# sailist/emotion-recognition-in-conversation

Measured on AMD Instinct MI355X. Metric: utterances/sec training step, COGMEN IEMOCAP-6 atv, higher is better.
Workload: dtype bf16

## Files before the change

emotion-recognition-in-conversation_amd/capi.py:

```python
import ctypes as C
import os
import re
import subprocess

import torch

_HERE = os.path.dirname(os.path.abspath(__file__))
LIB_PATH = os.environ.get("ERC_LIB_PATH") or os.path.join(_HERE, "lib", "libercgraft.so")
CSRC = os.path.join(_HERE, "csrc")
HEADER = os.path.join(os.path.dirname(_HERE), "include", "ercgraft.h")


class ErcGraftError(RuntimeError):
    pass


_CTYPES = {"int": C.c_int, "int32_t": C.c_int, "int64_t": C.c_int64, "uint64_t": C.c_uint64, "float": C.c_float}


def _ctype(decl, proto, ret=False):
    t = " ".join(decl.replace("*", " * ").split())
    if ret and t == "const char *":
        return C.c_char_p
    if "*" in t:
# ... 1100 lines not shown
    return list(order)[:n_nodes]


def chain_build(raw_graph):
    handle = int(lib().erc_chain_build(raw_graph))
    return (handle, None) if handle else (0, lib().erc_last_error().decode())


def chain_len(chain):
    n = int(lib().erc_chain_len(chain))
    if n < 0:
        _check(n, "erc_chain_len")
    return n


def chain_run(chain):
    _check(lib().erc_chain_run(chain, stream()), "erc_chain_run")


def chain_free(chain):
    _check(lib().erc_chain_free(chain), "erc_chain_free")
```

emotion-recognition-in-conversation_amd/csrc/cogmen_fused.hip:

```cpp
#include "erc_common.h"
#include "split_dev.h"

namespace {

typedef float f32x4 __attribute__((ext_vector_type(4)));
typedef short bf16x8 __attribute__((ext_vector_type(8)));

constexpr int CG_F = 100;
constexpr int CG_R = 8;
constexpr int CG_HL = 5;
constexpr int CG_TR = 16;
constexpr int CG_MID = CG_TR + 2 * CG_HL;
constexpr int CG_OUT = CG_TR + 4 * CG_HL;
constexpr int CG_FAR = CG_TR + 6 * CG_HL;
constexpr int CG_KM = (CG_R + 1) * CG_F;
constexpr int CG_KMP = 928;
constexpr int CG_SM = 936;
constexpr int CG_SH1 = 136;
constexpr int CG_SQ = 404;
constexpr int CG_CH = 12;
constexpr int CG_NT = 7;

constexpr int CG_NW = 16;
constexpr int CG_NTH = 64 * CG_NW;
// ... 103 lines not shown
    int* bn_counter;
    float* running_mean;
    float* running_var;
    float* saved;
    float momentum, eps, scale;
    int N, ldh0, ldmb, ldh1b, ldh2, bn_fused, two_spk;
    const int32_t* n_dev;
    int32_t* health;
    int32_t* events;
    uint64_t* stamps;
    int stamp_block;
    int64_t catT_plane, q_plane;
    float* Mf;
    float* H1f;
    int ldmf, ldh1f;
};

template <int NT>
__global__ __launch_bounds__(CG_NTH) void cogmen_fwd_tile_kernel(const CgFwdP p) {
    constexpr bool X = NT > 1;
    using XM = FxMap<X ? NT : 2>;
    if (p.health && blockIdx.x == 0 && threadIdx.x == 0 && *p.health != 0) {
        p.events[0] += 1;
        *p.health = 0;
    }
    extern __shared__ __attribute__((aligned(16))) unsigned char lds[];
    unsigned short* const sM = reinterpret_cast<unsigned short*>(lds + (X ? XM::SM_OFF : FW_SM_OFF));
    float* const sQ = reinterpret_cast<float*>(lds + (X ? XM::SM_OFF : FW_SM_OFF));
    unsigned short* const sH1 = reinterpret_cast<unsigned short*>(lds + (X ? XM::SH1_OFF : FW_SH1_OFF));
    float* const sH0 = reinterpret_cast<float*>(lds + (X ? XM::SH0_OFF : FW_SH0_OFF));
// ... 159 lines not shown
                            const int grp = (q >> 2) * 2 + (q & 1);
                            *reinterpret_cast<float2*>(grow + q * CG_F) = ((q >> 1) & 1) == a ? mq[grp] : make_float2(0.f, 0.f);
                        }
                        *reinterpret_cast<float2*>(grow + CG_R * CG_F) = self;
                    }
                }
            }
            uint32_t* const mrow = reinterpret_cast<uint32_t*>(sM + e * CG_SM);
            uint32_t* const grow = reinterpret_cast<uint32_t*>(p.Mb + (int64_t)(own ? node : 0) * p.ldmb);
            if (!X && act) {
#pragma unroll
                for (int q = 0; q < CG_R; ++q) {
                    const int grp = (q >> 2) * 2 + (q & 1);
                    const uint32_t v = ((q >> 1) & 1) == a ? pk4[grp] : 0u;
                    mrow[q * (CG_F / 2) + lane] = v;
                    if (own) grow[q * (CG_F / 2) + lane] = v;
                }
                mrow[CG_R * (CG_F / 2) + lane] = pks;
                if (own) grow[CG_R * (CG_F / 2) + lane] = pks;
            }
            if (own && lane < CG_R) {
                const int grp = (lane >> 2) * 2 + (lane & 1);
                int c = 0;
#pragma unroll
                for (int q = 0; q < 4; ++q) c = grp == q ? cnt[q] : c;
                c = ((lane >> 1) & 1) == a ? c : 0;
                p.inv_cnt[(int64_t)node * CG_R + lane] = c > 0 ? 1.0f / (float)c : 0.f;
            }
        }
    } else
    {
        const bool act = lane < CG_F / 2;
        const int c2 = 2 * min(lane, CG_F / 2 - 1);
#pragma unroll 1
// ... 24 lines not shown
            float2 self = *reinterpret_cast<const float2*>(sH0 + le * CG_F + c2);
            if (!valid) self = make_float2(0.f, 0.f);
            const bool own = valid && e >= CG_HL && e < CG_HL + CG_TR;
            uint32_t* const mrow = reinterpret_cast<uint32_t*>(sM + e * CG_SM);
            uint32_t* const grow = reinterpret_cast<uint32_t*>(p.Mb + (int64_t)(own ? node : 0) * p.ldmb);
            const float fc_l = (float)max(cnt_l, 1), rc_l = __builtin_amdgcn_rcpf(fc_l);
#pragma unroll
            for (int q = 0; q < CG_R; ++q) {
                const float fc = __builtin_bit_cast(float, __builtin_amdgcn_readlane(__builtin_bit_cast(int, fc_l), q));
                const float rc = __builtin_bit_cast(float, __builtin_amdgcn_readlane(__builtin_bit_cast(int, rc_l), q));
                float m0 = s0[q] * rc, m1 = s1[q] * rc;
                m0 = fmaf(fmaf(-m0, fc, s0[q]), rc, m0), m1 = fmaf(fmaf(-m1, fc, s1[q]), rc, m1);
                const uint32_t pk = (uint32_t)f2bf(m0) | ((uint32_t)f2bf(m1) << 16);
                if (act) {
                    mrow[q * (CG_F / 2) + lane] = pk;
                    if (own) grow[q * (CG_F / 2) + lane] = pk;
                }
            }
            const uint32_t pks = (uint32_t)f2bf(self.x) | ((uint32_t)f2bf(self.y) << 16);
            if (act) {
                mrow[CG_R * (CG_F / 2) + lane] = pks;
                if (own) grow[CG_R * (CG_F / 2) + lane] = pks;
            }
            if (own && lane < CG_R) p.inv_cnt[(int64_t)node * CG_R + lane] = cnt_l > 0 ? 1.0f / (float)cnt_l : 0.f;
        }
    }
    __syncthreads();
    CG_STAMP(2);

    f32x4 acc0 = {0.f, 0.f, 0.f, 0.f}, acc1 = {0.f, 0.f, 0.f, 0.f};
    if (mma_wave) {
        if constexpr (!X) {
            const unsigned short* const a0 = sM + r * CG_SM + 8 * g + 32 * KH0 * kh;
            const unsigned short* const a1 = sM + min(16 + r, 26) * CG_SM + 8 * g + 32 * KH0 * kh;
#pragma unroll
            for (int u = 0; u < KH0; ++u) {
                if (u < nkb) {
// ... 63 lines not shown
    if (mma_wave && !kh) {
        const float* src = sPart + (ct * 64 + lane) * 8;
        const f32x4 p0 = *reinterpret_cast<const f32x4*>(src), p1 = *reinterpret_cast<const f32x4*>(src + 4);
        const int col = 16 * ct + r;
        const float bias = p.b1[min(col, CG_F - 1)];
#pragma unroll
        for (int h = 0; h < 2; ++h)
#pragma unroll
            for (int i = 0; i < 4; ++i) {
                const int e = 16 * h + 4 * g + i;
                const float v = (h ? acc1[i] + p1[i] : acc0[i] + p0[i]) + bias;
                const int node = mb + e;
                if constexpr (!X) {
                    const unsigned short hb = col < CG_F ? f2bf(v) : (unsigned short)0;
                    sH1[e * CG_SH1 + col] = hb;
                    if (col < CG_F && e >= CG_HL && e < CG_HL + CG_TR && node < N) p.H1b[(int64_t)node * p.ldh1b + col] = hb;
                } else {
                    float rem = col < CG_F ? v : 0.f;
#pragma unroll
                    for (int t = 0; t < NT; ++t) {
                        const __bf16 hb = (__bf16)rem;
                        rem -= (float)hb;
                        sH1[t * (FW_SH1_BYTES / 2) + e * CG_SH1 + col] = __builtin_bit_cast(unsigned short, hb);
                    }
                    if (col < CG_F && e >= CG_HL && e < CG_HL + CG_TR && node < N) p.H1f[(int64_t)node * p.ldh1f + col] = v;
                }
            }
    } else if (w == 7) {
        for (int i = lane; i < 32 * 16 * NT; i += 64) sH1[(i >> 9) * (FW_SH1_BYTES / 2) + ((i >> 4) & 31) * CG_SH1 + 112 + (i & 15)] = 0;
    }
    __syncthreads();
    CG_STAMP(3);

    {
        bf16x8 fa[X ? 1 : 2][4];
        if constexpr (!X) {
#pragma unroll
            for (int h = 0; h < 2; ++h)
#pragma unroll
                for (int kb = 0; kb < 4; ++kb) fa[h][kb] = *reinterpret_cast<const bf16x8*>(sH1 + (16 * h + r) * CG_SH1 + 32 * kb + 8 * g);
        }
#pragma unroll
        for (int j = 0; j < 2; ++j) {
            const int qt = w + 16 * j;
            f32x4 acc[2] = {{0.f, 0.f, 0.f, 0.f}, {0.f, 0.f, 0.f, 0.f}};
            if constexpr (X) {
                const unsigned short* const bq1 = p.Wq + ((int64_t)min(w + 16, 24) * 4 * 64 + lane) * 8;
// ... 31 lines not shown
                        const int e = 16 * h + 4 * g + i;
                        if (e < CG_MID) sQ[e * CG_SQ + 16 * qt + r] = acc[h][i] + qbias[j];
                    }
            }
        }
    }
    __syncthreads();
    CG_STAMP(4);

#pragma unroll
    for (int j = 0; j < 2; ++j) {
        const int i = tid + CG_NTH * j;
        const int li = i / 100, q = i % 100;
        const int node = r0 + li;
        if (i < CG_TR * 100 && node < N)
            *reinterpret_cast<f32x4*>(p.QKVS + (int64_t)node * 400 + 4 * q) = *reinterpret_cast<const f32x4*>(sQ + (CG_HL + li) * CG_SQ + 4 * q);
    }

    {
        const bool act = lane < CG_F / 2;
        const int c2 = 2 * min(lane, CG_F / 2 - 1);
        const float am = act ? 1.f : 0.f;
        const int li = w, node = r0 + li, e = CG_HL + li;
        const bool valid = node < N;
        const int e0 = __builtin_amdgcn_readfirstlane(max(sIp[e] - E_lo, 0));
        const int nwin = __builtin_amdgcn_readfirstlane(valid ? min(max(sIp[e + 1] - sIp[e], 0), CG_CH) : 0);
        float2 qv = *reinterpret_cast<const float2*>(sQ + e * CG_SQ + c2);
        qv.x *= am, qv.y *= am;
        const float2 sk = *reinterpret_cast<const float2*>(sQ + e * CG_SQ + 3 * CG_F + c2);
        int ljs[CG_CH];
#pragma unroll
// ... 13 lines not shown
        for (int u = 0; u < CG_CH; ++u) {
            sc[u] *= p.scale;
            if (u < nwin) mx = fmaxf(mx, sc[u]);
        }
#pragma unroll
        for (int u = 0; u < CG_CH; ++u) {
            const float pw = u < nwin ? expf(sc[u] - mx) : 0.f;
            sc[u] = pw;
            den += pw;
            o0 += pw * vv[u].x, o1 += pw * vv[u].y;
        }
        const float inv = 1.0f / (den + 1e-16f);
        const float2 y = make_float2(valid ? o0 * inv + sk.x : 0.f, valid ? o1 * inv + sk.y : 0.f);
        if (act) *reinterpret_cast<float2*>(sH2 + li * CG_F + c2) = y;
        if (valid) {
            if (act) *reinterpret_cast<float2*>(p.H2 + (int64_t)node * p.ldh2 + c2) = y;
            float mine = 0.f;
#pragma unroll
            for (int u = 0; u < CG_CH; ++u)
                if (lane == u) mine = sc[u];
            if (lane < nwin) p.alpha[sIp[e] + lane] = mine * inv;
        }
    }
    CG_STAMP(5);
    if (!p.bn_fused) return;

    __syncthreads();
    if (tid < 2 * CG_F) {
        const int c = tid % CG_F, sq = tid / CG_F;
        double s = 0.0;
#pragma unroll
        for (int li = 0; li < CG_TR; ++li) {
            const double x = (double)sH2[li * CG_F + c];
            s += sq ? x * x : x;
        }
        if (p.bn_fused == 2) {
            reinterpret_cast<float*>(p.bn_part)[(int64_t)blockIdx.x * 2 * CG_F + tid] = (float)s;
        } else {
            st_sc1d(p.bn_part + (int64_t)blockIdx.x * 2 * CG_F + tid, s);
        }
    }
    if (p.bn_fused == 2) {
// ... 123 lines not shown
    float* dgamma;
    float* dbeta;
    float* stats;
    int head_parts, hp_floats;
    const unsigned short* WqT;
    const unsigned short* Wb;
    float* dQKVS;
    float* dH1;
    float* dH0;
    float scale;
    int N, ldh2, lddh0, lddh1, grads_bf16, two_spk;
    const int32_t* n_dev;
    uint64_t* stamps;
    int stamp_block;
    int64_t qT_plane, wb_plane;
};

template <int NT>
__global__ __launch_bounds__(CG_NTH) void cogmen_bwd_tile_kernel(const CgBwdP p) {
    constexpr bool X = NT > 1;
    using XM = BxMap<X ? NT : 2>;
    extern __shared__ __attribute__((aligned(16))) unsigned char lds[];
    float* const sK = reinterpret_cast<float*>(lds + (X ? XM::SK_OFF : BW_SK_OFF));
    float* const sV = reinterpret_cast<float*>(lds + (X ? XM::SV_OFF : BW_SV_OFF));
    float* const sQq = reinterpret_cast<float*>(lds + (X ? XM::SQ_OFF : BW_SQ_OFF));
    float* const sG = reinterpret_cast<float*>(lds + (X ? XM::SG_OFF : BW_SG_OFF));
    float* const sAl = reinterpret_cast<float*>(lds + (X ? XM::SE_OFF : BW_SE_OFF));
    int* const sSrc = reinterpret_cast<int*>(sAl + 2 * BW_ECAP);
    int* const sOd = sSrc + BW_ECAP;
    int* const sOt = sOd + 2 * BW_OCAP;
// ... 222 lines not shown
#pragma unroll
        for (int j = 0; j < 2; ++j) {
            const int i = tid + CG_NTH * j;
            const int em = i / 50, cp = i % 50;
            if (i < CG_MID * 50) {
                const float2 gv = *reinterpret_cast<const float2*>(sG + (em + CG_HL) * CG_F + 2 * cp);
                if constexpr (!X) {
                    sDQw[em * (CG_SDQ / 2) + 150 + cp] = (uint32_t)f2bf(gv.x) | ((uint32_t)f2bf(gv.y) << 16);
                } else {
                    unsigned tt[NT];
                    sp_split2<NT>(gv.x, gv.y, tt);
#pragma unroll
                    for (int t = 0; t < NT; ++t) sDQw[t * DQPW + em * (CG_SDQ / 2) + 150 + cp] = tt[t];
                }
                const int node = mb + em;
                if (em >= CG_HL && em < CG_HL + CG_TR && node < N) {
                    if (p.grads_bf16) *reinterpret_cast<uint32_t*>(reinterpret_cast<unsigned short*>(p.dQKVS) + (int64_t)node * 400 + 3 * CG_F + 2 * cp) = (uint32_t)f2bf(gv.x) | ((uint32_t)f2bf(gv.y) << 16);
                    else *reinterpret_cast<float2*>(p.dQKVS + (int64_t)node * 400 + 3 * CG_F + 2 * cp) = gv;
                }
            }
        }
#pragma unroll
        for (int ui = 0; ui < 3; ++ui) {
            if constexpr (!X) {
#pragma unroll
                for (int t5 = 0; t5 < 5; ++t5) bx[5 * ui + t5] = *reinterpret_cast<const bf16x8*>(brow5 + 512 * (5 * ui + t5));
            }
            const int u = w + CG_NW * ui;
            if (u >= 42) continue;
            const int kind = u < 14 ? 0 : 1 + (u - 14) / 14, uu = u < 14 ? u : (u - 14) % 14;
            const int rt = uu / 7, cti = uu % 7;
// ... 18 lines not shown
                const int node = mb + em;
                const bool rowv = em >= 0 && em < CG_MID;
                if (rowv && 16 * cti + r < CG_F) {
                    const bool nv = node >= 0 && node < N;
                    if constexpr (!X) {
                        sDQ[em * CG_SDQ + coff + 16 * cti + r] = f2bf(nv ? acc[q] : 0.f);
                    } else {
                        float rem = nv ? acc[q] : 0.f;
#pragma unroll
                        for (int t = 0; t < NT; ++t) {
                            const __bf16 hb = (__bf16)rem;
                            rem -= (float)hb;
                            sDQ[t * (BX_DQPLANE / 2) + em * CG_SDQ + coff + 16 * cti + r] = __builtin_bit_cast(unsigned short, hb);
                        }
                    }
                    if (nv && em >= CG_HL && em < CG_HL + CG_TR) {
                        if (p.grads_bf16) reinterpret_cast<unsigned short*>(p.dQKVS)[(int64_t)node * 400 + coff + 16 * cti + r] = f2bf(acc[q]);
                        else p.dQKVS[(int64_t)node * 400 + coff + 16 * cti + r] = acc[q];
                    }
                }
            }
        }
    }
    __syncthreads();
    CG_STAMP(3);

    {
        f32x4 acc0 = {0.f, 0.f, 0.f, 0.f}, acc1 = {0.f, 0.f, 0.f, 0.f};
        if (mma_wave) {
            const unsigned short* const a0 = sDQ + r * CG_SDQ + 8 * g + 32 * 7 * kh;
            if constexpr (!X) {
#pragma unroll
            for (int u = 0; u < 7; ++u) {
                if (u < (kh ? 6 : 7)) {
                    const bf16x8 fa0 = *reinterpret_cast<const bf16x8*>(a0 + 32 * u);
                    const bf16x8 fa1 = *reinterpret_cast<const bf16x8*>(a0 + 16 * CG_SDQ + 32 * u);
                    acc0 = __builtin_amdgcn_mfma_f32_16x16x32_bf16(fa0, fb3[u], acc0, 0, 0, 0);
                    acc1 = __builtin_amdgcn_mfma_f32_16x16x32_bf16(fa1, fb3[u], acc1, 0, 0, 0);
                }
            }
// ... 28 lines not shown
        }
        __syncthreads();
        if (mma_wave && !kh) {
            const float* src = sPart3 + (ct * 64 + lane) * 8;
            const f32x4 p0 = *reinterpret_cast<const f32x4*>(src), p1 = *reinterpret_cast<const f32x4*>(src + 4);
            const int col = 16 * ct + r;
            if (col < CG_F) {
#pragma unroll
                for (int h = 0; h < 2; ++h)
#pragma unroll
                    for (int i = 0; i < 4; ++i) {
                        const int e = 16 * h + 4 * g + i;
                        const float v = h ? acc1[i] + p1[i] : acc0[i] + p0[i];
                        sDH1[e * CG_F + col] = v;
                        const int node = mb + e;
                        if (e >= CG_HL && e < CG_HL + CG_TR && node < N) {
                            if (p.grads_bf16) reinterpret_cast<unsigned short*>(p.dH1)[(int64_t)node * p.lddh1 + col] = f2bf(v);
                            else p.dH1[(int64_t)node * p.lddh1 + col] = v;
                        }
                    }
            }
        }
    }
    __syncthreads();
    CG_STAMP(4);

    {
        const bool act = lane < CG_F / 2;
        const int c2 = 2 * min(lane, CG_F / 2 - 1);
        uint32_t* const sDPw = reinterpret_cast<uint32_t*>(sDP);
        const int li = w, em = CG_HL + li, node = r0 + li;
        const bool valid = node < N;
        const int o0 = __builtin_amdgcn_readfirstlane(sOp[em] - O_lo), o1 = __builtin_amdgcn_readfirstlane(sOp[em + 1] - O_lo);
        const int nwin = valid ? min(max(o1 - o0, 0), CG_CH) : 0;
        const int xb = max(o0, 0);
        const int xm = min(xb + min(lane, max(nwin - 1, 0)), BW_OCAP - 1);
        const int my_off = min(max(sOd[xm] - mb, 0), CG_MID - 1) * CG_F, my_typ = lane < nwin ? sOt[xm] : CG_R;
        const float my_w = sOw[xm];
        float s0[CG_R], s1[CG_R];
#pragma unroll
// ... 183 lines not shown
    p.Wq = (const unsigned short*)Wq; p.bq = bq; p.inv_cnt = inv_cnt;
    if (terms == 1) {
        p.Mb = (unsigned short*)Mb; p.H1b = (unsigned short*)H1b; p.ldmb = ldmb; p.ldh1b = ldh1b;
    } else {
        p.Mf = (float*)Mb; p.H1f = (float*)H1b; p.ldmf = ldmb; p.ldh1f = ldh1b; p.catT_plane = catT_plane; p.q_plane = q_plane;
    }
    p.QKVS = QKVS; p.H2 = H2; p.alpha = alpha;
    const int tiles = erc_cdiv(n_nodes, CG_TR);
    p.bn_part = bn_ws ? bn_ws + 2 : nullptr;
    p.bn_counter = reinterpret_cast<int*>(bn_ws);
    p.running_mean = running_mean; p.running_var = running_var; p.saved = saved;
    p.momentum = momentum; p.eps = eps; p.scale = scale;
    p.N = n_nodes; p.ldh0 = ldh0; p.ldh2 = ldh2; p.bn_fused = bn_fused;
    p.node_spk = node_spk; p.two_spk = n_speakers == 2 ? 1 : 0; p.n_dev = n_dev;
    p.health = health, p.events = events;
    p.stamps = g_cg_stamps; p.stamp_block = tiles / 2;
    if (terms == 1) hipLaunchKernelGGL(cogmen_fwd_tile_kernel<1>, dim3(tiles), dim3(CG_NTH), lds_bytes, (hipStream_t)stream, p);
    else if (terms == 2) hipLaunchKernelGGL(cogmen_fwd_tile_kernel<2>, dim3(tiles), dim3(CG_NTH), lds_bytes, (hipStream_t)stream, p);
    else hipLaunchKernelGGL(cogmen_fwd_tile_kernel<3>, dim3(tiles), dim3(CG_NTH), lds_bytes, (hipStream_t)stream, p);
    ERC_LAUNCH_CHECK("cogmen_fwd_tile");
    return ERC_OK;
}

extern "C" int erc_cogmen_fwd_tile(const float* H0, int ldh0, int n_nodes, int wp, int wf, const int32_t* in_ptr,
                                   const int32_t* in_src, const int32_t* in_typ, const void* WcatT, const float* b1,
                                   const void* Wq, const float* bq, float scale, void* Mb, int ldmb, float* inv_cnt, void* H1b,
                                   int ldh1b, float* QKVS, float* H2, int ldh2, float* alpha, int bn_fused,
                                   float* running_mean, float* running_var, float momentum, float eps, float* saved,
                                   double* bn_ws, const int32_t* node_spk, int n_speakers, const int32_t* n_dev, int32_t* health,
                                   int32_t* events, void* stream) {
// ... 41 lines not shown
    const void* kern = terms == 1 ? reinterpret_cast<const void*>(cogmen_bwd_tile_kernel<1>)
                     : terms == 2 ? reinterpret_cast<const void*>(cogmen_bwd_tile_kernel<2>)
                                  : reinterpret_cast<const void*>(cogmen_bwd_tile_kernel<3>);
    const int lds_bytes = terms == 1 ? BW_LDS : terms == 2 ? BxMap<2>::LDS : BxMap<3>::LDS;
    ERC_REQUIRE(ensure_lds(kern, lds_bytes), "cogmen_bwd_tile: %d bytes of LDS refused", lds_bytes);
    CgBwdP p{};
    p.dY = dY; p.H2 = H2; p.gamma = gamma; p.saved = saved; p.bn_bwd = bn_bwd; p.QKVS = QKVS; p.alpha = alpha;
    p.in_ptr = in_ptr; p.in_src = in_src; p.out_ptr = out_ptr; p.out_dst = out_dst; p.out_typ = out_typ; p.out_eid = out_eid;
    p.inv_cnt = inv_cnt; p.WqT = (const unsigned short*)WqT; p.Wb = (const unsigned short*)Wb;
    p.qT_plane = qT_plane; p.wb_plane = wb_plane;
    p.dQKVS = (float*)dQKVS; p.dH1 = (float*)dH1; p.dH0 = (float*)dH0; p.scale = scale; p.N = n_nodes; p.ldh2 = ldh2; p.lddh0 = lddh0;
    p.lddh1 = lddh1; p.grads_bf16 = grads_bf16;
    p.node_spk = node_spk; p.two_spk = n_speakers == 2 ? 1 : 0; p.n_dev = n_dev;
    p.head_part = head_part; p.head_parts = head_parts; p.hp_floats = head_part_floats; p.bn_bwd_out = const_cast<float*>(bn_bwd);
    p.dgamma = dgamma; p.dbeta = dbeta; p.stats = stats;
    p.stamps = g_cg_stamps; p.stamp_block = erc_cdiv(n_nodes, CG_TR) / 2;
    const dim3 grid(erc_cdiv(n_nodes, CG_TR));
    if (terms == 1) hipLaunchKernelGGL(cogmen_bwd_tile_kernel<1>, grid, dim3(CG_NTH), lds_bytes, (hipStream_t)stream, p);
    else if (terms == 2) hipLaunchKernelGGL(cogmen_bwd_tile_kernel<2>, grid, dim3(CG_NTH), lds_bytes, (hipStream_t)stream, p);
    else hipLaunchKernelGGL(cogmen_bwd_tile_kernel<3>, grid, dim3(CG_NTH), lds_bytes, (hipStream_t)stream, p);
    ERC_LAUNCH_CHECK("cogmen_bwd_tile");
    return ERC_OK;
}

extern "C" int erc_cogmen_bwd_tile(const float* dY, const float* H2, int ldh2, int n_nodes, int wp, int wf, const float* gamma,
                                   const float* saved, const float* bn_bwd, const float* QKVS, const float* alpha,
                                   const int32_t* in_ptr, const int32_t* in_src, const int32_t* out_ptr, const int32_t* out_dst,
                                   const int32_t* out_typ, const int32_t* out_eid, const float* inv_cnt, const void* WqT,
                                   const void* Wb, float scale, void* dQKVS, void* dH1, void* dH0, int lddh0,
                                   const int32_t* node_spk, int n_speakers, const float* head_part, int head_parts,
// ... 21 lines not shown
```

emotion-recognition-in-conversation_amd/csrc/launch_chain.hip:

```cpp
#include <dlfcn.h>

#include <vector>

#include "erc_common.h"

extern "C" int erc_chain_order(int n_nodes, int n_edges, const int32_t* from_host, const int32_t* to_host, int32_t* order_host) {
    ERC_REQUIRE(n_nodes > 0 && order_host != nullptr, "chain_order: n_nodes=%d (need >= 1 and an output array)", n_nodes);
    ERC_REQUIRE(n_edges == n_nodes - 1, "chain_order: %d nodes with %d edges are not one path", n_nodes, n_edges);
    ERC_REQUIRE(n_edges == 0 || (from_host != nullptr && to_host != nullptr), "chain_order: null edge list");
    std::vector<int32_t> next(n_nodes, -1), pred(n_nodes, -1);
    for (int e = 0; e < n_edges; ++e) {
        const int32_t a = from_host[e], b = to_host[e];
        ERC_REQUIRE(a >= 0 && a < n_nodes && b >= 0 && b < n_nodes && a != b, "chain_order: edge %d (%d -> %d) out of range", e, a, b);
        ERC_REQUIRE(next[a] < 0, "chain_order: node %d has two successors (a fork)", a);
        ERC_REQUIRE(pred[b] < 0, "chain_order: node %d has two predecessors (a join)", b);
        next[a] = b;
        pred[b] = a;
    }
    int root = -1, roots = 0;
    for (int i = 0; i < n_nodes; ++i)
        if (pred[i] < 0) {
            root = i;
            ++roots;
        }
// ... 104 lines not shown
            (void)hipGetLastError();
            return ERC_E_LAUNCH;
        }
    }
    return ERC_OK;
}

extern "C" int erc_chain_free(int64_t chain) {
    if (chain == 0) return ERC_OK;
    Chain* c = chain_of(chain);
    ERC_REQUIRE(c != nullptr, "chain_free: not a chain handle");
    c->magic = 0;
    delete c;
    return ERC_OK;
}
```

emotion-recognition-in-conversation_amd/csrc/wgrad_bf16.hip:

```cpp
#include "erc_common.h"
#include "optim_dev.h"
#include "split_dev.h"
#include <string.h>

namespace {

typedef float f32x4 __attribute__((ext_vector_type(4)));
typedef short bf16x8 __attribute__((ext_vector_type(8)));
typedef unsigned int u32x4 __attribute__((ext_vector_type(4)));
typedef unsigned int u32x2 __attribute__((ext_vector_type(2)));
#define ERC_GLOBAL __attribute__((address_space(1)))

constexpr int W2_IDX_CAP = 4096;
constexpr int W2_SLAB = 128 * 64 + 192;
constexpr int W2_MAX_DESC = 16;

struct W2Desc {
    const unsigned short* A;
    const unsigned short* B;
    float* C;
    float* bias_a;
    float* bias_b;
    const int32_t* b_gather;
    const int32_t* k_dev;
    int lda, ldb, ldc, M, N, K;
    int ct, cvec, splits, tiles_n, item_base, n_items, tile_base;
    int kind;
};

struct W2Adam {
    int decoupled, spin_limit;
    float lr, b1, b2, eps, wd, grad_scale;
    float *data, *grad, *m, *v;
    int64_t* state;
    unsigned short* shadow;
    const int32_t* skip;
    int32_t* seq;
    int32_t* health;
    ShadowTab tab;
    int x_world, x_rank, x_spin, x_pad;
    float* x_pub[8];
    int32_t* x_flags[8];
    int64_t* x_epoch;
    int64_t x_npad;
};
static_assert(sizeof(W2Desc) == 112, "W2Desc layout");

__device__ __forceinline__ float ld_sc1(const float* p) { return __hip_atomic_load(p, __ATOMIC_RELAXED, __HIP_MEMORY_SCOPE_AGENT); }
__device__ __forceinline__ void st_sc1(float* p, float v) { __hip_atomic_store(p, v, __ATOMIC_RELAXED, __HIP_MEMORY_SCOPE_AGENT); }
__device__ __forceinline__ void st_sc1_x4(float* p, f32x4 v) {
    asm volatile("global_store_dwordx4 %0, %1, off sc0 sc1\n\ts_nop 1" ::"v"(p), "v"(v) : "memory");
}
__device__ __forceinline__ f32x4 ld_sc1_x4(const float* p) {
    f32x4 v;
    asm volatile("global_load_dwordx4 %0, %1, off sc0 sc1" : "=v"(v) : "v"(p) : "memory");
    return v;
}
__device__ __forceinline__ float bf_lo(unsigned d) { return __builtin_bit_cast(float, d << 16); }
__device__ __forceinline__ float bf_hi(unsigned d) { return __builtin_bit_cast(float, d & 0xffff0000u); }
__device__ __forceinline__ unsigned perm_lo(unsigned x, unsigned y) { return __builtin_amdgcn_perm(y, x, 0x05040100u); }
__device__ __forceinline__ unsigned perm_hi(unsigned x, unsigned y) { return __builtin_amdgcn_perm(y, x, 0x07060302u); }

#define W2_STAMP(slot)                                                                          \
    do {                                                                                        \
        if (stamps && threadIdx.x == 0) stamps[slot] = __builtin_amdgcn_s_memrealtime();        \
    } while (0)

// ... 24 lines not shown
    auto copy_tab = [&]() __attribute__((always_inline)) {
        ShadowTab* const wt = reinterpret_cast<ShadowTab*>(red);
        wt->n = ad.tab.n, wt->flags = ad.tab.flags;
#pragma unroll
        for (int t = 0; t < SHADOW_MAX; ++t) {
            const ShadowDesc& a = ad.tab.d[t];
            ShadowDesc& b = wt->d[t];
            b.src_off = a.src_off, b.n_el = a.n_el, b.dst_off = a.dst_off, b.n0 = a.n0, b.n1 = a.n1, b.sn0 = a.sn0, b.sn1 = a.sn1;
            b.sn2 = a.sn2, b.sk0 = a.sk0, b.sk1 = a.sk1, b.sk2 = a.sk2, b.ld = a.ld, b.mode = a.mode;
            b.plane_stride = a.plane_stride, b.terms = a.terms;
        }
    };
    auto adam_quad = [&](const int64_t off, const f32x4 gq, const f32x4 pq, const f32x4 mq, const f32x4 vq) __attribute__((always_inline)) -> float4 {
        float4 pv = make_float4(pq.x, pq.y, pq.z, pq.w), mv = make_float4(mq.x, mq.y, mq.z, mq.w), vv = make_float4(vq.x, vq.y, vq.z, vq.w);
        ac.upd(pv.x, gq.x, mv.x, vv.x), ac.upd(pv.y, gq.y, mv.y, vv.y), ac.upd(pv.z, gq.z, mv.z, vv.z), ac.upd(pv.w, gq.w, mv.w, vv.w);
        *(ERC_GLOBAL f32x4*)(ad.data + off) = (f32x4){pv.x, pv.y, pv.z, pv.w};
        *(ERC_GLOBAL f32x4*)(ad.m + off) = (f32x4){mv.x, mv.y, mv.z, mv.w}, *(ERC_GLOBAL f32x4*)(ad.v + off) = (f32x4){vv.x, vv.y, vv.z, vv.w};
        return pv;
    };
    auto shadow_quads = [&](const int64_t (&offs)[8], const float4 (&pn)[8], const int count, const bool (&isq)[8], const unsigned tmask) __attribute__((always_inline)) {
        if (!ad.shadow) return;
        const bool quads = (stab.flags & 1) != 0;
        const int nt = stab.n;
#pragma unroll
        for (int o = 0; o < 8; ++o) {
            if (o >= count || !isq[o]) continue;
            const int64_t i0 = offs[o];
            const float4 pv = pn[o];
#pragma unroll 1
            for (int t = 0; t < nt; ++t) {
                if (!((tmask >> t) & 1)) continue;
                const ShadowDesc& sd = stab.d[t];
// ... 410 lines not shown
                        *reinterpret_cast<f32x4*>(red + w * 4096 + (((hh * 2 + il) * 4 + q) * 64 + lane) * 4) = v * wsel;
                    }
            __syncthreads();
    #pragma unroll
            for (int u = 0; u < 4; ++u) {
                const int f4 = tid + 256 * u;
                f32x4 s = *reinterpret_cast<const f32x4*>(red + f4 * 4);
    #pragma unroll
                for (int ww = 1; ww < 4; ++ww) {
                    const f32x4 t = *reinterpret_cast<const f32x4*>(red + ww * 4096 + f4 * 4);
                    s += t;
                }
                if (direct) {
                    store_c(tid + 256 * (u & 1), 2 * P + (u >> 1), s);
                } else {
                    st_sc1_x4(slab + ((4 * P + u) * 256 + tid) * 4, s);
                }
            }
        }
        if (tid < 192) {
            const float v = ((bred[tid] + bred[192 + tid]) + bred[384 + tid]) + bred[576 + tid];
            if (direct) {
                if (tid < 128) {
                    if (want_a && tid < d.M) ((ERC_GLOBAL float*)d.bias_a)[tid] = v;
                } else if (want_b && n0 + tid - 128 < d.N) {
                    ((ERC_GLOBAL float*)d.bias_b)[n0 + tid - 128] = v;
                }
            } else {
                st_sc1(slab + 8192 + tid, v);
            }
        }
// ... 92 lines not shown
    #pragma unroll
                for (int o = 1; o < 8; ++o) res[o] = z;
            }
            W2_STAMP(9);
            float bsum = 0.f;
#pragma unroll
            for (int jj = 0; jj < 8; ++jj) bsum += bt[jj] * (jj < S ? 1.f : 0.f);
            if (ad.x_world > 1) {
                const int64_t poff = x_poff();
                float* mypub = nullptr;
#pragma unroll
                for (int r = 0; r < 8; ++r)
                    if (r == ad.x_rank) mypub = ad.x_pub[r];
#pragma unroll
                for (int o = 0; o < 8; ++o)
                    if (o < owned && valid[o] == 4) st_sc1_x4(mypub + poff + off[o], res[o]);
                if (bdst) __hip_atomic_store(mypub + poff + boff, bsum, __ATOMIC_RELAXED, __HIP_MEMORY_SCOPE_SYSTEM);
                adam_on = x_rendezvous(!adam_on) && adam_on;
                bump_step();
                if (adam_on) {
#pragma unroll
                    for (int o = 0; o < 8; ++o)
                        if (o < owned && valid[o] == 4) res[o] = x_sum4(poff + off[o]);
                    if (bdst) bsum = x_sum1(poff + boff);
                }
            }
            const bool upd = adam_on;
            unsigned tmask = 0;
            {
                const int64_t lo = cbase, hi = cbase + (int64_t)(ct ? d.N : d.M) * d.ldc;
                const int nt = stab.n;
                for (int t = 0; t < nt; ++t)
                    if (stab.d[t].src_off < hi && stab.d[t].src_off + stab.d[t].n_el > lo) tmask |= 1u << t;
            }
    #pragma unroll 1
            for (int it = 0; it < owned; ++it) {
                if (valid[0] == 4) {
                    *(ERC_GLOBAL f32x4*)(ad.grad + off[0]) = res[0];
                    if (upd) {
                        const float4 pv = adam_quad(off[0], res[0], pq[0], mq[0], vq[0]);
                        if (it == 0) W2_STAMP(13);
                        if (ad.shadow) {
                            const int nt = stab.n;
    #pragma unroll 1
                            for (int t = 0; t < nt; ++t) {
                                if (!((tmask >> t) & 1)) continue;
                                shadow_store4_desc(ad.shadow, stab.d[t], (stab.flags & (2 << t)) != 0, off[0], pv);
                            }
                        }
                    }
                } else if (valid[0] != 0) {
                    __hip_atomic_store(ad.health, ERC_HEALTH_RAISED, __ATOMIC_RELAXED, __HIP_MEMORY_SCOPE_AGENT);
                }
// ... 180 lines not shown

static int w2_adam_entry(int terms, const void* table, int n_desc, const int32_t* item_base, int n_items, float* slabs,
                         int32_t* counters, int n_tiles, float* p, float* g, float* m, float* v, int64_t n, float lr,
                         float beta1, float beta2, float eps, float weight_decay, int decoupled, float grad_scale,
                         int64_t* state, void* shadow_base, int64_t shadow_numel, const ErcShadowTab* tab_host,
                         int32_t* health, void* stream, const ErcP2P* x = nullptr) {
    static_assert(sizeof(ShadowTab) == sizeof(ErcShadowTab), "shadow table layout");
    ERC_REQUIRE(p && g && m && v && state && health && n > 0 && n_tiles >= 0 && n_items <= 256,
                "wgrad_bf16_adam: bad arguments (at most 256 work items: all of them must be resident)");
    ERC_REQUIRE((((uintptr_t)p | (uintptr_t)g | (uintptr_t)m | (uintptr_t)v) & 15) == 0, "wgrad_bf16_adam: 16-byte alignment");
    W2Adam ad{};
    ad.decoupled = decoupled, ad.lr = lr, ad.b1 = beta1, ad.b2 = beta2, ad.eps = eps, ad.wd = weight_decay;
    ad.grad_scale = grad_scale, ad.data = p, ad.grad = g, ad.m = m, ad.v = v, ad.state = state, ad.skip = health, ad.health = health;
    ad.seq = counters + n_tiles;
    ad.spin_limit = g_w2_spin_limit;
    if (x) {
        ERC_REQUIRE(x->world >= 2 && x->world <= 8 && x->rank >= 0 && x->rank < x->world && x->epoch && x->n_pad >= n && x->n_pad % 4 == 0 &&
                        (int32_t*)x->health == health, "wgrad_adam_p2p: bad exchange descriptor (2 <= world <= 8; health = the exchange's health word)");
        ad.x_world = x->world, ad.x_rank = x->rank, ad.x_spin = x->spin_limit > 0 ? x->spin_limit : 4000000;
        ad.x_epoch = (int64_t*)x->epoch, ad.x_npad = x->n_pad;
        for (int r = 0; r < x->world; ++r) {
            ERC_REQUIRE(x->pub[r] && x->flags[r] && ((uintptr_t)x->pub[r] & 15) == 0, "wgrad_adam_p2p: peer %d not mapped", r);
            ad.x_pub[r] = (float*)x->pub[r], ad.x_flags[r] = (int32_t*)x->flags[r];
        }
    }
    if (tab_host) memcpy(&ad.tab, tab_host, sizeof(ad.tab));
    ERC_REQUIRE(ad.tab.n == 0 || shadow_base, "wgrad_bf16_adam: shadow table without a shadow buffer");
    ERC_REQUIRE(ad.tab.n >= 0 && ad.tab.n <= SHADOW_MAX, "wgrad_bf16_adam: %d shadow descriptors", ad.tab.n);
    ad.tab.flags = ad.tab.n > 0;
    for (int t = 0; t < ad.tab.n; ++t) {
// ... 48 lines not shown
```

emotion-recognition-in-conversation_amd/engine.py:

```python
import math
import os

import torch

from . import capi

ALIGN = 64


class WorkspaceCache:

    def __init__(self, maxsize=None):
        import collections
        self.maxsize = int(os.environ.get("ERC_WS_CACHE", 4)) if maxsize is None else maxsize
        self._d = collections.OrderedDict()
        self.last = None

    def get(self, key, make):
        ws = self._d.get(key)
        if ws is None:
            ws = make()
            self._d[key] = ws
            while len(self._d) > self.maxsize:
                victim = next((k for k in self._d if k != key), None)
# ... 555 lines not shown
            self.side._dirty = True

    def __exit__(self, *exc):
        if self.side.enabled:
            self.ctx.__exit__(*exc)
        return False


def step_replay_mode():
    mode = os.environ.get("ERC_STEP_REPLAY", "") or "auto"
    if mode not in ("auto", "graph", "launches"):
        raise capi.ErcGraftError("ERC_STEP_REPLAY=%s: expected 'graph' or 'launches'" % mode)
    return mode


class CapturedStep:

    def __init__(self, fn, steps=1, mode=None):
        self.mode = mode or step_replay_mode()
        self.chain, self.refused = 0, None
        keep = self.mode != "graph"
        self.graph = torch.cuda.CUDAGraph(keep_graph=True) if keep else torch.cuda.CUDAGraph()
        with torch.cuda.graph(self.graph):
            for _ in range(steps):
                self.out = fn()
        if keep:
            self.chain, self.refused = capi.chain_build(self.graph.raw_cuda_graph())
            if not self.chain:
                if self.mode == "launches":
                    raise capi.ErcGraftError("ERC_STEP_REPLAY=launches: the captured step cannot be replayed as plain launches: %s"
                                             % self.refused)
                self.graph.instantiate()
        self.launches = capi.chain_len(self.chain) if self.chain else None
        self._run = capi.lib().erc_chain_run if self.chain else None
# ... 43 lines not shown
```

include/ercgraft.h:

```cpp
#ifndef ERCGRAFT_H
#define ERCGRAFT_H

#include <stdint.h>

#ifdef __cplusplus
extern "C" {
#endif

#define ERC_ABI_VERSION 3

#define ERC_OK 0
#define ERC_E_ARG (-1)
#define ERC_E_LAUNCH (-2)

int erc_abi_version(void);
const char* erc_last_error(void);

int erc_window_graph_build(const int64_t* lengths, const int64_t* speakers, int64_t spk_sb, int64_t spk_st,
                           int B, int T, int wp, int wf, int n_speakers, int n_cap, int e_cap,
                           int32_t* node_off, int32_t* node_row, int32_t* node_spk,
                           int32_t* in_ptr, int32_t* in_src, int32_t* in_typ,
                           int32_t* out_ptr, int32_t* out_dst, int32_t* out_typ, int32_t* out_eid,
                           int64_t* edge_index, int64_t* edge_type, int32_t* counts, void* stream);
int erc_window_graph_build_desc(const int64_t* lengths, const int64_t* speakers, int64_t spk_sb, int64_t spk_st,
// ... 548 lines not shown
                           const int32_t* node_off, const int32_t* node_spk, int B, int T, int S, int64_t N, float drop_p,
                           float drop_rec, const uint64_t* rng_state, uint64_t rng_stream, const float* save,
                           const float* dEmo, int ldde, float* dGX, int lddgx, float* dREC, void* stream);
int erc_bcrnn_meta_cap(const int64_t* lengths, const int32_t* desc, const int64_t* store_label, int zero_store_row, int B, int T,
                       int n_cap, int32_t* node_off, int32_t* node_row, int32_t* pad_node, int32_t* x_row, int64_t* label_out,
                       int32_t* counts, void* stream);
int erc_log_softmax_rows(const float* x, int ldx, int C, int n_rows, float* y, int ldy, void* stream);


int erc_chain_order(int n_nodes, int n_edges, const int32_t* from_host, const int32_t* to_host, int32_t* order_host);
int64_t erc_chain_build(void* graph_host);
int erc_chain_len(int64_t chain);
int erc_chain_run(int64_t chain, void* stream);
int erc_chain_free(int64_t chain);

int erc_test_poison_lds(int32_t* sink, void* stream);

#ifdef __cplusplus
}
#endif
#endif
```

Measured before the change: 22.57 million.

## Stage tile outputs through LDS and store rows with write-through dwordx4

Forward and backward COGMEN tile kernels now write their M, H1, H2, dQKVS and dH1 tiles as coalesced 16-byte row pieces read from LDS after a barrier, replacing scattered per-lane global stores. A new store helper can issue write-through stores (sc0 sc1), and a global store mode that defaults to write-through is applied to these outputs and to the wgrad/Adam parameter, moment and gradient writes. The aim is fewer, wider store transactions and making data visible to the next kernel in the chain sooner. The trade-off is extra post-barrier store phases and possible cache-bypass costs.

```diff
diff --git a/emotion-recognition-in-conversation_amd/capi.py b/emotion-recognition-in-conversation_amd/capi.py
--- a/emotion-recognition-in-conversation_amd/capi.py
+++ b/emotion-recognition-in-conversation_amd/capi.py
@@ -1138,6 +1138,10 @@
     return n
 
 
+def set_store_mode(through):
+    _call("erc_set_store_mode", 1 if through else 0)
+
+
 def chain_run(chain):
     _check(lib().erc_chain_run(chain, stream()), "erc_chain_run")
 
diff --git a/emotion-recognition-in-conversation_amd/csrc/cogmen_fused.hip b/emotion-recognition-in-conversation_amd/csrc/cogmen_fused.hip
--- a/emotion-recognition-in-conversation_amd/csrc/cogmen_fused.hip
+++ b/emotion-recognition-in-conversation_amd/csrc/cogmen_fused.hip
@@ -1,5 +1,6 @@
 #include "erc_common.h"
 #include "split_dev.h"
+#include "store_dev.h"
 
 namespace {
 
@@ -141,6 +142,7 @@
     float* Mf;
     float* H1f;
     int ldmf, ldh1f;
+    int wt, mb_rows, h1_rows, h2_rows;
 };
 
 template <int NT>
@@ -330,10 +332,10 @@
                     const int grp = (q >> 2) * 2 + (q & 1);
                     const uint32_t v = ((q >> 1) & 1) == a ? pk4[grp] : 0u;
                     mrow[q * (CG_F / 2) + lane] = v;
-                    if (own) grow[q * (CG_F / 2) + lane] = v;
+                    if (own && !p.mb_rows) grow[q * (CG_F / 2) + lane] = v;
                 }
                 mrow[CG_R * (CG_F / 2) + lane] = pks;
-                if (own) grow[CG_R * (CG_F / 2) + lane] = pks;
+                if (own && !p.mb_rows) grow[CG_R * (CG_F / 2) + lane] = pks;
             }
             if (own && lane < CG_R) {
                 const int grp = (lane >> 2) * 2 + (lane & 1);
@@ -388,13 +390,13 @@
                 const uint32_t pk = (uint32_t)f2bf(m0) | ((uint32_t)f2bf(m1) << 16);
                 if (act) {
                     mrow[q * (CG_F / 2) + lane] = pk;
-                    if (own) grow[q * (CG_F / 2) + lane] = pk;
+                    if (own && !p.mb_rows) grow[q * (CG_F / 2) + lane] = pk;
                 }
             }
             const uint32_t pks = (uint32_t)f2bf(self.x) | ((uint32_t)f2bf(self.y) << 16);
             if (act) {
                 mrow[CG_R * (CG_F / 2) + lane] = pks;
-                if (own) grow[CG_R * (CG_F / 2) + lane] = pks;
+                if (own && !p.mb_rows) grow[CG_R * (CG_F / 2) + lane] = pks;
             }
             if (own && lane < CG_R) p.inv_cnt[(int64_t)node * CG_R + lane] = cnt_l > 0 ? 1.0f / (float)cnt_l : 0.f;
         }
@@ -488,7 +490,7 @@
                 if constexpr (!X) {
                     const unsigned short hb = col < CG_F ? f2bf(v) : (unsigned short)0;
                     sH1[e * CG_SH1 + col] = hb;
-                    if (col < CG_F && e >= CG_HL && e < CG_HL + CG_TR && node < N) p.H1b[(int64_t)node * p.ldh1b + col] = hb;
+                    if (!p.h1_rows && col < CG_F && e >= CG_HL && e < CG_HL + CG_TR && node < N) p.H1b[(int64_t)node * p.ldh1b + col] = hb;
                 } else {
                     float rem = col < CG_F ? v : 0.f;
 #pragma unroll
@@ -502,9 +504,33 @@
             }
     } else if (w == 7) {
         for (int i = lane; i < 32 * 16 * NT; i += 64) sH1[(i >> 9) * (FW_SH1_BYTES / 2) + ((i >> 4) & 31) * CG_SH1 + 112 + (i & 15)] = 0;
+    } else if (!X && w >= 8) {
+        if (p.mb_rows) {
+            constexpr int PCS = (CG_KM * 2 + 15) / 16;
+            static_assert(PCS * 8 <= CG_SM && CG_TR * PCS <= 4 * 512 && (CG_SM * 2) % 16 == 0, "row pieces of the M tile");
+#pragma unroll
+            for (int j = 0; j < 4; ++j) {
+                const int i = tid - 512 + 512 * j;
+                const int li = i / PCS, q = i % PCS;
+                const int node = r0 + li;
+                if (i < CG_TR * PCS && node < N)
+                    st_out16(p.Mb + (int64_t)node * p.ldmb + 8 * q, *reinterpret_cast<const f32x4*>(sM + (CG_HL + li) * CG_SM + 8 * q), p.wt);
+            }
+        }
     }
     __syncthreads();
     CG_STAMP(3);
+
+    if constexpr (!X) {
+        if (p.h1_rows) {
+            constexpr int PCS = (CG_F * 2 + 15) / 16;
+            static_assert(PCS * 8 <= CG_SH1 && CG_TR * PCS <= CG_NTH && (CG_SH1 * 2) % 16 == 0, "row pieces of the H1 tile");
+            const int li = tid / PCS, q = tid % PCS;
+            const int node = r0 + li;
+            if (tid < CG_TR * PCS && node < N)
+                st_out16(p.H1b + (int64_t)node * p.ldh1b + 8 * q, *reinterpret_cast<const f32x4*>(sH1 + (CG_HL + li) * CG_SH1 + 8 * q), p.wt);
+        }
+    }
 
     {
         bf16x8 fa[X ? 1 : 2][4];
@@ -566,7 +592,7 @@
         const int li = i / 100, q = i % 100;
         const int node = r0 + li;
         if (i < CG_TR * 100 && node < N)
-            *reinterpret_cast<f32x4*>(p.QKVS + (int64_t)node * 400 + 4 * q) = *reinterpret_cast<const f32x4*>(sQ + (CG_HL + li) * CG_SQ + 4 * q);
+            st_out16(p.QKVS + (int64_t)node * 400 + 4 * q, *reinterpret_cast<const f32x4*>(sQ + (CG_HL + li) * CG_SQ + 4 * q), p.wt);
     }
 
     {
@@ -610,7 +636,7 @@
         const float2 y = make_float2(valid ? o0 * inv + sk.x : 0.f, valid ? o1 * inv + sk.y : 0.f);
         if (act) *reinterpret_cast<float2*>(sH2 + li * CG_F + c2) = y;
         if (valid) {
-            if (act) *reinterpret_cast<float2*>(p.H2 + (int64_t)node * p.ldh2 + c2) = y;
+            if (act && !p.h2_rows) *reinterpret_cast<float2*>(p.H2 + (int64_t)node * p.ldh2 + c2) = y;
             float mine = 0.f;
 #pragma unroll
             for (int u = 0; u < CG_CH; ++u)
@@ -622,6 +648,11 @@
     if (!p.bn_fused) return;
 
     __syncthreads();
+    if (p.h2_rows && tid >= 512 && tid < 512 + CG_TR * (CG_F / 4)) {
+        const int li = (tid - 512) / (CG_F / 4), q = (tid - 512) % (CG_F / 4);
+        const int node = r0 + li;
+        if (node < N) st_out16(p.H2 + (int64_t)node * p.ldh2 + 4 * q, *reinterpret_cast<const f32x4*>(sH2 + li * CG_F + 4 * q), p.wt);
+    }
     if (tid < 2 * CG_F) {
         const int c = tid % CG_F, sq = tid / CG_F;
         double s = 0.0;
@@ -775,6 +806,7 @@
     uint64_t* stamps;
     int stamp_block;
     int64_t qT_plane, wb_plane;
+    int wt, dq_rows, dh1_rows;
 };
 
 template <int NT>
@@ -1027,7 +1059,7 @@
                     for (int t = 0; t < NT; ++t) sDQw[t * DQPW + em * (CG_SDQ / 2) + 150 + cp] = tt[t];
                 }
                 const int node = mb + em;
-                if (em >= CG_HL && em < CG_HL + CG_TR && node < N) {
+                if ((X || !p.dq_rows) && em >= CG_HL && em < CG_HL + CG_TR && node < N) {
                     if (p.grads_bf16) *reinterpret_cast<uint32_t*>(reinterpret_cast<unsigned short*>(p.dQKVS) + (int64_t)node * 400 + 3 * CG_F + 2 * cp) = (uint32_t)f2bf(gv.x) | ((uint32_t)f2bf(gv.y) << 16);
                     else *reinterpret_cast<float2*>(p.dQKVS + (int64_t)node * 400 + 3 * CG_F + 2 * cp) = gv;
                 }
@@ -1076,7 +1108,7 @@
                             sDQ[t * (BX_DQPLANE / 2) + em * CG_SDQ + coff + 16 * cti + r] = __builtin_bit_cast(unsigned short, hb);
                         }
                     }
-                    if (nv && em >= CG_HL && em < CG_HL + CG_TR) {
+                    if ((X || !p.dq_rows) && nv && em >= CG_HL && em < CG_HL + CG_TR) {
                         if (p.grads_bf16) reinterpret_cast<unsigned short*>(p.dQKVS)[(int64_t)node * 400 + coff + 16 * cti + r] = f2bf(acc[q]);
                         else p.dQKVS[(int64_t)node * 400 + coff + 16 * cti + r] = acc[q];
                     }
@@ -1086,6 +1118,17 @@
     }
     __syncthreads();
     CG_STAMP(3);
+
+    if constexpr (!X) {
+        if (p.dq_rows && tid < CG_TR * 50) {
+            static_assert((CG_SDQ * 2) % 16 == 0 && CG_TR * 50 <= CG_NTH, "row pieces of the dQKVS tile");
+            const int li = tid / 50, q = tid % 50;
+            const int node = r0 + li;
+            if (node < N)
+                st_out16(reinterpret_cast<unsigned short*>(p.dQKVS) + (int64_t)node * 400 + 8 * q,
+                         *reinterpret_cast<const f32x4*>(sDQ + (CG_HL + li) * CG_SDQ + 8 * q), p.wt);
+        }
+    }
 
     {
         f32x4 acc0 = {0.f, 0.f, 0.f, 0.f}, acc1 = {0.f, 0.f, 0.f, 0.f};
@@ -1144,7 +1187,7 @@
                         const float v = h ? acc1[i] + p1[i] : acc0[i] + p0[i];
                         sDH1[e * CG_F + col] = v;
                         const int node = mb + e;
-                        if (e >= CG_HL && e < CG_HL + CG_TR && node < N) {
+                        if ((X || !p.dh1_rows) && e >= CG_HL && e < CG_HL + CG_TR && node < N) {
                             if (p.grads_bf16) reinterpret_cast<unsigned short*>(p.dH1)[(int64_t)node * p.lddh1 + col] = f2bf(v);
                             else p.dH1[(int64_t)node * p.lddh1 + col] = v;
                         }
@@ -1154,6 +1197,22 @@
     }
     __syncthreads();
     CG_STAMP(4);
+
+    if constexpr (!X) {
+        if (p.dh1_rows && tid < CG_TR * 13) {
+            const int li = tid / 13, q = tid % 13;
+            const int node = r0 + li;
+            const float* const src = sDH1 + (CG_HL + li) * CG_F + 8 * q;
+            const f32x4 lo = *reinterpret_cast<const f32x4*>(src);
+            f32x4 hi = {0.f, 0.f, 0.f, 0.f};
+            if (q < 12) hi = *reinterpret_cast<const f32x4*>(src + 4);
+            const uint32_t d0 = (uint32_t)f2bf(lo[0]) | ((uint32_t)f2bf(lo[1]) << 16), d1 = (uint32_t)f2bf(lo[2]) | ((uint32_t)f2bf(lo[3]) << 16);
+            const uint32_t d2 = (uint32_t)f2bf(hi[0]) | ((uint32_t)f2bf(hi[1]) << 16), d3 = (uint32_t)f2bf(hi[2]) | ((uint32_t)f2bf(hi[3]) << 16);
+            if (node < N)
+                st_out16(reinterpret_cast<unsigned short*>(p.dH1) + (int64_t)node * p.lddh1 + 8 * q,
+                         (f32x4){__builtin_bit_cast(float, d0), __builtin_bit_cast(float, d1), __builtin_bit_cast(float, d2), __builtin_bit_cast(float, d3)}, p.wt);
+        }
+    }
 
     {
         const bool act = lane < CG_F / 2;
@@ -1367,6 +1426,10 @@
     p.N = n_nodes; p.ldh0 = ldh0; p.ldh2 = ldh2; p.bn_fused = bn_fused;
     p.node_spk = node_spk; p.two_spk = n_speakers == 2 ? 1 : 0; p.n_dev = n_dev;
     p.health = health, p.events = events;
+    p.wt = erc_store_mode();
+    p.mb_rows = terms == 1 && ldmb % 8 == 0 && ldmb >= 8 * ((CG_KM + 7) / 8) && ((uintptr_t)Mb & 15) == 0;
+    p.h1_rows = terms == 1 && ldh1b % 8 == 0 && ldh1b >= 8 * ((CG_F + 7) / 8) && ((uintptr_t)H1b & 15) == 0;
+    p.h2_rows = bn_fused != 0 && ldh2 % 4 == 0 && ((uintptr_t)H2 & 15) == 0;
     p.stamps = g_cg_stamps; p.stamp_block = tiles / 2;
     if (terms == 1) hipLaunchKernelGGL(cogmen_fwd_tile_kernel<1>, dim3(tiles), dim3(CG_NTH), lds_bytes, (hipStream_t)stream, p);
     else if (terms == 2) hipLaunchKernelGGL(cogmen_fwd_tile_kernel<2>, dim3(tiles), dim3(CG_NTH), lds_bytes, (hipStream_t)stream, p);
@@ -1438,6 +1501,9 @@
     p.node_spk = node_spk; p.two_spk = n_speakers == 2 ? 1 : 0; p.n_dev = n_dev;
     p.head_part = head_part; p.head_parts = head_parts; p.hp_floats = head_part_floats; p.bn_bwd_out = const_cast<float*>(bn_bwd);
     p.dgamma = dgamma; p.dbeta = dbeta; p.stats = stats;
+    p.wt = erc_store_mode();
+    p.dq_rows = terms == 1 && grads_bf16 && ((uintptr_t)dQKVS & 15) == 0;
+    p.dh1_rows = terms == 1 && grads_bf16 && lddh1 % 8 == 0 && lddh1 >= 8 * ((CG_F + 7) / 8) && ((uintptr_t)dH1 & 15) == 0;
     p.stamps = g_cg_stamps; p.stamp_block = erc_cdiv(n_nodes, CG_TR) / 2;
     const dim3 grid(erc_cdiv(n_nodes, CG_TR));
     if (terms == 1) hipLaunchKernelGGL(cogmen_bwd_tile_kernel<1>, grid, dim3(CG_NTH), lds_bytes, (hipStream_t)stream, p);
diff --git a/emotion-recognition-in-conversation_amd/csrc/launch_chain.hip b/emotion-recognition-in-conversation_amd/csrc/launch_chain.hip
--- a/emotion-recognition-in-conversation_amd/csrc/launch_chain.hip
+++ b/emotion-recognition-in-conversation_amd/csrc/launch_chain.hip
@@ -3,6 +3,7 @@
 #include <vector>
 
 #include "erc_common.h"
+#include "store_dev.h"
 
 extern "C" int erc_chain_order(int n_nodes, int n_edges, const int32_t* from_host, const int32_t* to_host, int32_t* order_host) {
     ERC_REQUIRE(n_nodes > 0 && order_host != nullptr, "chain_order: n_nodes=%d (need >= 1 and an output array)", n_nodes);
@@ -142,3 +143,11 @@
     delete c;
     return ERC_OK;
 }
+
+static int g_store_mode = 1;
+int erc_store_mode(void) { return g_store_mode; }
+extern "C" int erc_set_store_mode(int mode) {
+    ERC_REQUIRE(mode == 0 || mode == 1, "set_store_mode: mode = %d (0 plain, 1 write-through)", mode);
+    g_store_mode = mode;
+    return ERC_OK;
+}
diff --git a/emotion-recognition-in-conversation_amd/csrc/store_dev.h b/emotion-recognition-in-conversation_amd/csrc/store_dev.h
--- /dev/null
+++ b/emotion-recognition-in-conversation_amd/csrc/store_dev.h
@@ -0,0 +1,21 @@
+#pragma once
+#include "erc_common.h"
+
+int erc_store_mode(void);
+
+#ifdef __HIPCC__
+typedef float st_f32x4 __attribute__((ext_vector_type(4)));
+
+template <bool WT>
+__device__ __forceinline__ void st_out16(void* p, const st_f32x4 v) {
+    if constexpr (WT) {
+        asm volatile("global_store_dwordx4 %0, %1, off sc0 sc1\n\ts_nop 1" ::"v"(p), "v"(v) : "memory");
+    } else {
+        *(__attribute__((address_space(1))) st_f32x4*)p = v;
+    }
+}
+__device__ __forceinline__ void st_out16(void* p, const st_f32x4 v, const int wt) {
+    if (wt) st_out16<true>(p, v);
+    else st_out16<false>(p, v);
+}
+#endif
diff --git a/emotion-recognition-in-conversation_amd/csrc/wgrad_bf16.hip b/emotion-recognition-in-conversation_amd/csrc/wgrad_bf16.hip
--- a/emotion-recognition-in-conversation_amd/csrc/wgrad_bf16.hip
+++ b/emotion-recognition-in-conversation_amd/csrc/wgrad_bf16.hip
@@ -1,6 +1,7 @@
 #include "erc_common.h"
 #include "optim_dev.h"
 #include "split_dev.h"
+#include "store_dev.h"
 #include <string.h>
 
 namespace {
@@ -38,7 +39,8 @@
     int32_t* seq;
     int32_t* health;
     ShadowTab tab;
-    int x_world, x_rank, x_spin, x_pad;
+    int x_world, x_rank, x_spin;
+    int wt;
     float* x_pub[8];
     int32_t* x_flags[8];
     int64_t* x_epoch;
@@ -48,9 +50,6 @@
 
 __device__ __forceinline__ float ld_sc1(const float* p) { return __hip_atomic_load(p, __ATOMIC_RELAXED, __HIP_MEMORY_SCOPE_AGENT); }
 __device__ __forceinline__ void st_sc1(float* p, float v) { __hip_atomic_store(p, v, __ATOMIC_RELAXED, __HIP_MEMORY_SCOPE_AGENT); }
-__device__ __forceinline__ void st_sc1_x4(float* p, f32x4 v) {
-    asm volatile("global_store_dwordx4 %0, %1, off sc0 sc1\n\ts_nop 1" ::"v"(p), "v"(v) : "memory");
-}
 __device__ __forceinline__ f32x4 ld_sc1_x4(const float* p) {
     f32x4 v;
     asm volatile("global_load_dwordx4 %0, %1, off sc0 sc1" : "=v"(v) : "v"(p) : "memory");
@@ -105,8 +104,13 @@
     auto adam_quad = [&](const int64_t off, const f32x4 gq, const f32x4 pq, const f32x4 mq, const f32x4 vq) __attribute__((always_inline)) -> float4 {
         float4 pv = make_float4(pq.x, pq.y, pq.z, pq.w), mv = make_float4(mq.x, mq.y, mq.z, mq.w), vv = make_float4(vq.x, vq.y, vq.z, vq.w);
         ac.upd(pv.x, gq.x, mv.x, vv.x), ac.upd(pv.y, gq.y, mv.y, vv.y), ac.upd(pv.z, gq.z, mv.z, vv.z), ac.upd(pv.w, gq.w, mv.w, vv.w);
-        *(ERC_GLOBAL f32x4*)(ad.data + off) = (f32x4){pv.x, pv.y, pv.z, pv.w};
-        *(ERC_GLOBAL f32x4*)(ad.m + off) = (f32x4){mv.x, mv.y, mv.z, mv.w}, *(ERC_GLOBAL f32x4*)(ad.v + off) = (f32x4){vv.x, vv.y, vv.z, vv.w};
+        if (NT == 1 && ad.wt) {
+            st_out16<true>(ad.data + off, (f32x4){pv.x, pv.y, pv.z, pv.w});
+            st_out16<true>(ad.m + off, (f32x4){mv.x, mv.y, mv.z, mv.w}), st_out16<true>(ad.v + off, (f32x4){vv.x, vv.y, vv.z, vv.w});
+        } else {
+            *(ERC_GLOBAL f32x4*)(ad.data + off) = (f32x4){pv.x, pv.y, pv.z, pv.w};
+            *(ERC_GLOBAL f32x4*)(ad.m + off) = (f32x4){mv.x, mv.y, mv.z, mv.w}, *(ERC_GLOBAL f32x4*)(ad.v + off) = (f32x4){vv.x, vv.y, vv.z, vv.w};
+        }
         return pv;
     };
     auto shadow_quads = [&](const int64_t (&offs)[8], const float4 (&pn)[8], const int count, const bool (&isq)[8], const unsigned tmask) __attribute__((always_inline)) {
@@ -547,7 +551,7 @@
                 if (direct) {
                     store_c(tid + 256 * (u & 1), 2 * P + (u >> 1), s);
                 } else {
-                    st_sc1_x4(slab + ((4 * P + u) * 256 + tid) * 4, s);
+                    st_out16<true>(slab + ((4 * P + u) * 256 + tid) * 4, s);
                 }
             }
         }
@@ -670,7 +674,7 @@
                     if (r == ad.x_rank) mypub = ad.x_pub[r];
 #pragma unroll
                 for (int o = 0; o < 8; ++o)
-                    if (o < owned && valid[o] == 4) st_sc1_x4(mypub + poff + off[o], res[o]);
+                    if (o < owned && valid[o] == 4) st_out16<true>(mypub + poff + off[o], res[o]);
                 if (bdst) __hip_atomic_store(mypub + poff + boff, bsum, __ATOMIC_RELAXED, __HIP_MEMORY_SCOPE_SYSTEM);
                 adam_on = x_rendezvous(!adam_on) && adam_on;
                 bump_step();
@@ -692,7 +696,8 @@
     #pragma unroll 1
             for (int it = 0; it < owned; ++it) {
                 if (valid[0] == 4) {
-                    *(ERC_GLOBAL f32x4*)(ad.grad + off[0]) = res[0];
+                    if (NT == 1 && ad.wt) st_out16<true>(ad.grad + off[0], res[0]);
+                    else *(ERC_GLOBAL f32x4*)(ad.grad + off[0]) = res[0];
                     if (upd) {
                         const float4 pv = adam_quad(off[0], res[0], pq[0], mq[0], vq[0]);
                         if (it == 0) W2_STAMP(13);
@@ -903,6 +908,7 @@
     ad.grad_scale = grad_scale, ad.data = p, ad.grad = g, ad.m = m, ad.v = v, ad.state = state, ad.skip = health, ad.health = health;
     ad.seq = counters + n_tiles;
     ad.spin_limit = g_w2_spin_limit;
+    ad.wt = (x || terms > 1) ? 0 : erc_store_mode();
     if (x) {
         ERC_REQUIRE(x->world >= 2 && x->world <= 8 && x->rank >= 0 && x->rank < x->world && x->epoch && x->n_pad >= n && x->n_pad % 4 == 0 &&
                         (int32_t*)x->health == health, "wgrad_adam_p2p: bad exchange descriptor (2 <= world <= 8; health = the exchange's health word)");
diff --git a/emotion-recognition-in-conversation_amd/engine.py b/emotion-recognition-in-conversation_amd/engine.py
--- a/emotion-recognition-in-conversation_amd/engine.py
+++ b/emotion-recognition-in-conversation_amd/engine.py
@@ -593,10 +593,19 @@
     return mode
 
 
+def step_store_mode():
+    mode = os.environ.get("ERC_STEP_STORES", "") or "through"
+    if mode not in ("plain", "through"):
+        raise capi.ErcGraftError("ERC_STEP_STORES=%s: expected 'plain' or 'through'" % mode)
+    return mode
+
+
 class CapturedStep:
 
     def __init__(self, fn, steps=1, mode=None):
         self.mode = mode or step_replay_mode()
+        self.stores = step_store_mode()
+        capi.set_store_mode(self.stores == "through")
         self.chain, self.refused = 0, None
         keep = self.mode != "graph"
         self.graph = torch.cuda.CUDAGraph(keep_graph=True) if keep else torch.cuda.CUDAGraph()
diff --git a/include/ercgraft.h b/include/ercgraft.h
--- a/include/ercgraft.h
+++ b/include/ercgraft.h
@@ -586,6 +586,8 @@
 int erc_chain_run(int64_t chain, void* stream);
 int erc_chain_free(int64_t chain);
 
+int erc_set_store_mode(int mode);
+
 int erc_test_poison_lds(int32_t* sink, void* stream);
 
 #ifdef __cplusplus
```

Result: faster. 23.13 million (median of 6 runs) (+2.5%).
